# pierrepaleo/sift_pyocl

Hardware: AMD Instinct MI355X
Metric: SiftPlan.keypoints throughput, 4096x4096 fp32 (Mpix/s; keypoints/s in keypoints_per_s) (higher is better)
Workload: dtype f32

## Files before the change

sift_pyocl_amd/csrc/k_keypoint.hpp:

```cpp
#pragma once
#include <hip/hip_runtime.h>
#include <stdint.h>
#include "k_extrema.hpp"
#include "siftmath.hpp"

namespace siftk {

struct KpRecord { float x, y, scale, angle; uint8_t desc[128]; };
static_assert(sizeof(KpRecord) == 144, "record layout");

struct GradTaps { float xa, xb, ya, yb; bool bx, by; };

__device__ __forceinline__ GradTaps gradient_fetch(const float *__restrict__ I, int x, int y, int W, int H) {
    const size_t pos = (size_t)y * W + x;
    GradTaps t;
    t.bx = (x == 0) || (x == W - 1);
    t.by = (y == 0) || (y == H - 1);
    t.xa = I[x == W - 1 ? pos : pos + 1];
    t.xb = I[x == 0 ? pos : pos - 1];
    t.ya = I[y == 0 ? pos : pos - W];
    t.yb = I[y == H - 1 ? pos : pos + W];
    return t;
}

__device__ __forceinline__ void gradient_eval(const GradTaps &t, float &mag, float &ori) {
    float gx = t.xa - t.xb, gy = t.ya - t.yb;
    if (t.bx) gx = 2.0f * gx;
    if (t.by) gy = 2.0f * gy;
    mag = sqrtf(gx * gx + gy * gy);
    ori = siftmath::atan2f_(-gy, gx);
}

__device__ __forceinline__ void gradient_at(const float *__restrict__ I, int x, int y, int W, int H,
                                            float &mag, float &ori) {
    gradient_eval(gradient_fetch(I, x, y, W, H), mag, ori);
}

__device__ __forceinline__ int div_exact(int idx, int d, float inv, int &rem) {
    int q = (int)((float)idx * inv);
    rem = idx - q * d;
    if (rem < 0) { q--; rem += d; }
    else if (rem >= d) { q++; rem -= d; }
    return q;
}

#define SIFT_MAX_OCTAVES 24
#define SIFT_GROUPS 3
struct Counters {
    int n_rec;
    int tail_timeout;
    unsigned rec_word[SIFT_GROUPS];
    int g_kp[SIFT_GROUPS];
    int g_out[SIFT_GROUPS];
    int desc_next[SIFT_GROUPS];
    int n_cand[SIFT_MAX_OCTAVES + 1];
    int c_scale[SIFT_MAX_OCTAVES][3];
    int o_scale[SIFT_MAX_OCTAVES][3];
    uint32_t mm[2];
    int tail_ready[8];
};

struct OctaveTable {
    const float *base;
    long long off[SIFT_MAX_OCTAVES];
    int W[SIFT_MAX_OCTAVES], H[SIFT_MAX_OCTAVES];
    const float *gmap, *omap;
};
__device__ __forceinline__ size_t map_offset(const OctaveTable &tab, int oct, int scale) {
    return (size_t)(tab.off[oct] / 2) + (size_t)(scale - 1) * tab.W[oct] * tab.H[oct];
}

struct alignas(16) RecordSink {
    KpRecord *dev, *host;
    int dev_limit, host_limit;
};

__device__ __forceinline__ void descriptor_open(Counters *cnt, int group, int n, KpRecord *records, int rec_capacity, KpRecord *host_records,
                                                int host_capacity, RecordSink *S) {
    if (threadIdx.x == 0) {
        int base = 0;
        if (cnt) {
            if (blockIdx.x == 0) {
                base = atomicAdd(&cnt->n_rec, n);
                __hip_atomic_store(&cnt->rec_word[group], 0x80000000u | (unsigned)base, __ATOMIC_RELAXED, __HIP_MEMORY_SCOPE_AGENT);
            } else {
                unsigned w;
                while (!((w = __hip_atomic_load(&cnt->rec_word[group], __ATOMIC_RELAXED, __HIP_MEMORY_SCOPE_AGENT)) & 0x80000000u)) __builtin_amdgcn_s_sleep(16);
                base = (int)(w & 0x7fffffffu);
            }
        }
        S->dev = records + base; S->dev_limit = rec_capacity - base;
        S->host = host_records ? host_records + base : nullptr; S->host_limit = host_records ? host_capacity - base : 0;
    }
    __syncthreads();
}

__device__ __forceinline__ void store_record(const RecordSink *S, int i, const float4 kq, int b0, int b1, int lane, unsigned char *bytes) {
    bytes[lane] = (unsigned char)b0; bytes[lane + 64] = (unsigned char)b1;
    __builtin_amdgcn_wave_barrier();
    unsigned w = 0u;
    if (lane < 4) w = __float_as_uint(lane == 0 ? kq.x : (lane == 1 ? kq.y : (lane == 2 ? kq.z : kq.w)));
    else if (lane < 36) w = reinterpret_cast<const unsigned *>(bytes)[lane - 4];
    if (lane < 36) {
        const volatile RecordSink *v = S;
        if (i < v->dev_limit) reinterpret_cast<unsigned *>(v->dev + i)[lane] = w;
        if (i < v->host_limit) reinterpret_cast<unsigned *>(v->host + i)[lane] = w;
    }
    __builtin_amdgcn_wave_barrier();
}

__global__ void gather_records_kernel(const KpRecord *__restrict__ records, const int *__restrict__ idx, KpRecord *__restrict__ out, int n) {
    const long long total = (long long)n * 36;
    for (long long t = (long long)blockIdx.x * blockDim.x + threadIdx.x; t < total; t += (long long)gridDim.x * blockDim.x) {
        const int j = (int)(t / 36), w = (int)(t - (long long)j * 36);
        reinterpret_cast<unsigned *>(out + j)[w] = reinterpret_cast<const unsigned *>(records + idx[j])[w];
    }
}

#ifdef SIFT_PHASE_CLOCK
__device__ unsigned long long g_phase[32];
struct PhaseClock {
    unsigned long long t, t0;
    unsigned long long *acc;
    __device__ __forceinline__ void start(unsigned long long *lds16, int lane) {
        acc = lds16;
        if (lane < 16) lds16[lane] = 0ull;
        __builtin_amdgcn_wave_barrier();
        t0 = t = __builtin_amdgcn_s_memtime();
    }
    __device__ __forceinline__ void mark(int k, int lane) {
        const unsigned long long now = __builtin_amdgcn_s_memtime();
        if (lane == 0) (void)__hip_atomic_fetch_add(acc + k, now - t, __ATOMIC_RELAXED, __HIP_MEMORY_SCOPE_WORKGROUP);
        t = now;
    }
    __device__ __forceinline__ void count(int k, int lane) { if (lane == 0) (void)__hip_atomic_fetch_add(acc + k, 1ull, __ATOMIC_RELAXED, __HIP_MEMORY_SCOPE_WORKGROUP); }
    __device__ __forceinline__ void flush(int base, int lane) {
        const unsigned long long now = __builtin_amdgcn_s_memtime();
        if (lane == 0) acc[12] = now - t0;
        __builtin_amdgcn_wave_barrier();
        if (lane < 15) atomicAdd(&g_phase[base + lane], acc[lane]);
        if (lane == 15) atomicMax(&g_phase[base + 15], acc[12]);
    }
};
#define PH_MARK(k) ph.mark((k), lane)
#define PH_COUNT(k) ph.count((k), lane)
#define PH_WAIT_VM(n) asm volatile("s_waitcnt vmcnt(" #n ")" ::: "memory")
#else
#define PH_MARK(k)
#define PH_COUNT(k)
#define PH_WAIT_VM(n)
#endif

#define ABL(x) false

#define SIFT_ORI_OBUF 96
struct alignas(16) OriWaveLds {
    float pool[64 + 36 * 3 + 4];
    uint2 mask[36];
    unsigned mbase[36];
    float4 obuf[SIFT_ORI_OBUF];
    int oaux[SIFT_ORI_OBUF];
#ifdef SIFT_PHASE_CLOCK
    unsigned long long ph[16];
#endif
};

__device__ __forceinline__ int wave_prefix_incl(int x) {
    int t = x;
    t += __builtin_amdgcn_update_dpp(0, t, 0x111, 0xf, 0xf, false);
    t += __builtin_amdgcn_update_dpp(0, t, 0x112, 0xf, 0xf, false);
    t += __builtin_amdgcn_update_dpp(0, t, 0x114, 0xf, 0xf, false);
    t += __builtin_amdgcn_update_dpp(0, t, 0x118, 0xf, 0xf, false);
    t += __builtin_amdgcn_update_dpp(0, t, 0x142, 0xa, 0xf, false);
    t += __builtin_amdgcn_update_dpp(0, t, 0x143, 0xc, 0xf, false);
    return t;
}

template <bool MAPS>
__global__ __launch_bounds__(256) void orientation_kernel(OctaveTable tab, float ori_sigma,
                                                          const float4 *__restrict__ kp,
                                                          const int *__restrict__ kp_aux, Counters *cnt, int group,
                                                          int kp_capacity, float4 *__restrict__ okp,
                                                          int *__restrict__ oaux, int out_capacity, int team_below, int small_blocks) {
    __shared__ OriWaveLds lds_all[4];
    __shared__ double fold[36];
    __shared__ int s_hist[3 * SIFT_MAX_OCTAVES];
    const int lane = threadIdx.x & 63;
    OriWaveLds &L = lds_all[threadIdx.x >> 6];
    const int n = min(cnt->g_kp[group], kp_capacity);
    const int first = 0;
    const int count = n - first;
    const int nblocks = min((int)gridDim.x, count < 16384 ? small_blocks : (count < 65536 ? max(1024, small_blocks) : 4096));
    if ((int)blockIdx.x >= nblocks) return;
#ifdef SIFT_PHASE_CLOCK
    PhaseClock ph;
    ph.start(L.ph, lane);
#endif
    siftmath::load_atan_fold(fold);
    if (lane < 36) L.mask[lane] = make_uint2(0u, 0u);
    if (threadIdx.x < 3 * SIFT_MAX_OCTAVES) s_hist[threadIdx.x] = 0;
    __syncthreads();
    PH_MARK(0);
    const int wave = (blockIdx.x * blockDim.x + threadIdx.x) >> 6;
    const int nwaves = (nblocks * blockDim.x) >> 6;
    const float4 *pool4 = reinterpret_cast<const float4 *>(L.pool);
    __shared__ int s_pending[4], s_base;
    int pending = 0;
    auto store_pending = [&](int slot, int count) {
        __builtin_amdgcn_wave_barrier();
        for (int e = lane; e < count; e += 64)
            if (slot + e < out_capacity) { okp[slot + e] = L.obuf[e]; oaux[slot + e] = L.oaux[e]; }
        __builtin_amdgcn_wave_barrier();
    };
    auto flush_wave = [&]() {
        int slot = 0;
        if (lane == 0) slot = atomicAdd(&cnt->g_out[group], pending);
        store_pending(__shfl(slot, 0), pending);
        pending = 0;
    };
    const bool team = count < team_below;
    const int w4 = threadIdx.x >> 6;
    const int boff = team ? 64 * w4 : 0, bstep = team ? 256 : 64;
    for (int i = first + (team ? (int)blockIdx.x : wave); i < n; i += (team ? nblocks : nwaves)) {
        const float4 k = kp[i];
        const int aux = __builtin_amdgcn_readfirstlane(kp_aux[i]);
        const int scale = aux & 0xff, oct = aux >> 8;
        const int W = tab.W[oct], H = tab.H[oct], octsize = 1 << oct;
        if (!(k.y >= 0.0f)) continue;
        const float *I = tab.base + tab.off[oct] + (size_t)scale * W * H;
        const float *Gm = MAPS ? tab.gmap + map_offset(tab, oct, scale) : nullptr;
        const float *Om = MAPS ? tab.omap + map_offset(tab, oct, scale) : nullptr;
        auto taps_at = [&](int x, int y) {
            if (!MAPS) return gradient_fetch(I, x, y, W, H);
            GradTaps t = {};
            const size_t pos = (size_t)y * W + x;
            t.xa = Gm[pos]; t.xb = Om[pos];
            return t;
        };
        const int row = (int)((double)k.y + 0.5), col = (int)((double)k.z + 0.5);
        const float sigma = ori_sigma * k.w;
        const int radius = (int)((double)sigma * 3.0);
        const int rmin = max(0, row - radius), cmin = max(0, col - radius);
        const int rmax = min(row + radius, H - 2), cmax = min(col + radius, W - 2);
        const float lim = (float)(radius * radius) + 0.5f;
        const float two_s2 = 2.0f * sigma * sigma;
        const float r_two_s2 = 1.0f / two_s2;
        const bool fast_div = two_s2 >= 1e-3f && two_s2 <= 1e6f;
        const int wc = cmax - cmin + 1, hr = rmax - rmin + 1;
        const int total = (wc > 0 && hr > 0) ? wc * hr : 0;
        const float inv_wc = 1.0f / (float)max(wc, 1);
        float h = 0.0f;
        auto locate = [&](int base, int &r, int &c) {
            const int idx = base + lane;
            if (idx >= total) return false;
            int rem;
            const int q = div_exact(idx, wc, inv_wc, rem);
            r = rmin + q; c = cmin + rem;
            return true;
        };
        int nr = 0, nc = 0;
        bool nvalid = locate(boff, nr, nc);
        GradTaps ntaps = {};
        if (nvalid) ntaps = taps_at(nc, nr);
        PH_COUNT(13);
        PH_MARK(1);
        for (int base = 0; base < total; base += bstep) {
            bool valid = nvalid;
            const int r = nr, c = nc;
            const GradTaps taps = ntaps;
            nvalid = locate(base + bstep + boff, nr, nc);
            if (nvalid) ntaps = taps_at(nc, nr);
#ifdef SIFT_PHASE_CLOCK
            PH_COUNT(14);
            if (base + bstep + boff < total) PH_WAIT_VM(4); else PH_WAIT_VM(0);
            PH_MARK(2);
#endif
            int bin = 0;
            float val = 0.0f;
            if (valid) {
                float gx = taps.xa - taps.xb, gy = taps.ya - taps.yb;
                if (taps.bx) gx = 2.0f * gx;
                if (taps.by) gy = 2.0f * gy;
                const float gval = MAPS ? taps.xa : sqrtf(gx * gx + gy * gy);
                float dif = (float)r - k.y;
                float distsq = dif * dif;
                dif = (float)c - k.z;
                distsq = distsq + dif * dif;
                valid = (gval > 0.0f) && (distsq < lim);
                if (valid) {
                    const float earg = fast_div ? siftmath::div_by_reciprocal(-distsq, two_s2, r_two_s2) : -distsq / two_s2;
                    bool ok_a = true, ok_e;
                    float a = MAPS ? taps.xb : siftmath::atan2f_fast_try(-gy, gx, fold, ok_a);
                    float ew = siftmath::expf_fast_try(earg, ok_e);
                    if (!(ok_a && ok_e)) {
                        if (!MAPS && !ok_a) a = siftmath::atan2f_(-gy, gx);
                        if (!ok_e) ew = siftmath::expf_(earg);
                    }
                    bin = (int)siftmath::div_by_reciprocal(36.0f * (a + SM_PI_F + 0.001f), 2.0f * SM_PI_F, 1.0f / (2.0f * SM_PI_F));
                    valid = (bin >= 0) && (bin <= 36);
                    bin = min(max(bin, 0), 35);
                    val = ew * gval;
                }
                if (valid) atomicOr(reinterpret_cast<unsigned *>(L.mask) + 2 * bin + (lane >> 5), 1u << (lane & 31));
            }
            __builtin_amdgcn_wave_barrier();
            PH_MARK(3);
            const uint2 mine = (lane < 36) ? L.mask[lane] : make_uint2(0u, 0u);
            const int votes = __popc(mine.x) + __popc(mine.y);
            const int padded = (votes + 3) & ~3;
            const int seg = wave_prefix_incl(padded) - padded;
            if (lane < 36) L.mbase[lane] = (unsigned)seg;
            if (votes) reinterpret_cast<float4 *>(L.pool)[(seg + padded - 4) >> 2] = make_float4(0.f, 0.f, 0.f, 0.f);
            __builtin_amdgcn_wave_barrier();
            PH_MARK(4);
            {
                const uint2 mk = L.mask[bin];
                const unsigned mb = L.mbase[bin];
                const int pos = mb + __builtin_amdgcn_mbcnt_hi(mk.y, __builtin_amdgcn_mbcnt_lo(mk.x, 0u));
                if (valid) L.pool[pos] = val;
            }
            __builtin_amdgcn_wave_barrier();
            PH_MARK(5);
            if (!team) {
                for (int k0 = 0; k0 < padded; k0 += 4) {
                    const float4 v = pool4[(seg + k0) >> 2];
                    h = h + v.x; h = h + v.y; h = h + v.z; h = h + v.w;
                }
                if (votes) L.mask[lane] = make_uint2(0u, 0u);
                __builtin_amdgcn_wave_barrier();
                PH_MARK(6);
            } else {
                __syncthreads();
                if (w4 == 0 && lane < 36) {
#pragma unroll
                    for (int q = 0; q < 4; q++) {
                        const uint2 mq = lds_all[q].mask[lane];
                        const int vq = __popc(mq.x) + __popc(mq.y);
                        const int sq = (int)lds_all[q].mbase[lane];
                        const float4 *pq = reinterpret_cast<const float4 *>(lds_all[q].pool);
                        for (int k0 = 0; k0 < vq; k0 += 4) {
                            const float4 v = pq[(sq + k0) >> 2];
                            h = h + v.x; h = h + v.y; h = h + v.z; h = h + v.w;
                        }
                        if (vq) lds_all[q].mask[lane] = make_uint2(0u, 0u);
                    }
                }
                __syncthreads();
            }
        }
        if (team && w4 != 0) continue;
        const int lp = (lane == 0) ? 35 : lane - 1, ln = (lane >= 35) ? 0 : lane + 1;
        auto third = [&](float s) {
            return (__builtin_fabsf(s) >= 1e-25f && __builtin_fabsf(s) <= 1e30f) ? siftmath::div_by_reciprocal(s, 3.0f, 1.0f / 3.0f)
                                                                            : (float)((double)s / 3.0);
        };
#pragma unroll 1
        for (int pass = 0; pass < 6; pass++) {
            const float prev = __shfl(h, lp), nxt = __shfl(h, ln);
            float nh = third((prev + h) + nxt);
            const float nh0 = __shfl(nh, 0);
            if (lane == 35) nh = third((prev + h) + nh0);
            h = (lane < 36) ? nh : 0.0f;
        }
        float mx = (lane < 36) ? h : 0.0f;
#pragma unroll
        for (int off = 32; off > 0; off >>= 1) mx = fmaxf(mx, __shfl_xor(mx, off));
        const float maxval = fmaxf(mx, 0.0f);
        const uint64_t eq = __ballot(lane < 36 && h == maxval);
        const int argmax = (maxval > 0.0f && eq) ? (__ffsll((unsigned long long)eq) - 1) : 0;
        const float hp = __shfl(h, argmax == 0 ? 35 : argmax - 1);
        const float hn = __shfl(h, argmax == 35 ? 0 : argmax + 1);
        const float interp = 0.5f * (hp - hn) / (hp - 2.0f * maxval + hn);
        const float angle = 2.0f * SM_PI_F * ((float)argmax + 0.5f + interp) / 36.0f - SM_PI_F;
        const float hpp = __shfl(h, lp), hnn = __shfl(h, ln);
        bool extra = (lane < 36) && h > hpp && h > hnn && h >= 0.8f * maxval && lane != argmax;
        float a2 = 0.0f;
        if (extra) {
            const float it = 0.5f * (hpp - hnn) / (hpp - 2.0f * h + hnn);
            a2 = (float)((double)(2.0f * SM_PI_F * ((float)lane + 0.5f + it)) / 36.0 - (double)SM_PI_F);
            extra = (a2 >= -SM_PI_F) && (a2 <= SM_PI_F);
        }
        const uint64_t emask = __ballot(extra);
        const float ox = k.z * (float)octsize, oy = k.y * (float)octsize, os = k.w * (float)octsize;
        const float sum4 = ((ox + oy) + os) + angle;
        const int nmain = (sum4 == sum4) ? 1 : 0;
        const int nextra = __popcll((unsigned long long)emask);
        if (lane == 0) atomicAdd(&s_hist[3 * oct + min(max(scale - 1, 0), 2)], 1 + nextra);
        if (pending + nmain + nextra > SIFT_ORI_OBUF) flush_wave();
        if (lane == 0 && nmain) { L.obuf[pending] = make_float4(ox, oy, os, angle); L.oaux[pending] = aux; }
        if (extra) {
            const int at = pending + nmain + __popcll((unsigned long long)(emask & ((1ull << lane) - 1ull)));
            L.obuf[at] = make_float4(ox, oy, os, a2);
            L.oaux[at] = aux;
        }
        pending += nmain + nextra;
        PH_MARK(7);
    }
    if (lane == 0) s_pending[threadIdx.x >> 6] = pending;
    __syncthreads();
    if (threadIdx.x == 0) {
        const int tot = s_pending[0] + s_pending[1] + s_pending[2] + s_pending[3];
        s_base = tot ? atomicAdd(&cnt->g_out[group], tot) : 0;
    }
    __syncthreads();
    {
        const int w = threadIdx.x >> 6;
        int slot = s_base;
        for (int q = 0; q < w; q++) slot += s_pending[q];
        store_pending(slot, pending);
    }
    for (int t = threadIdx.x; t < 3 * SIFT_MAX_OCTAVES; t += blockDim.x)
        if (s_hist[t]) atomicAdd(&cnt->o_scale[0][0] + t, s_hist[t]);
#ifdef SIFT_PHASE_CLOCK
    PH_MARK(8);
    ph.flush(0, lane);
#endif
}


struct DescWaveLds {
    unsigned int mlo[128], mhi[128], mbase[128];
    float pool[8 * 64];
    int pool_cnt;
    int sij[128];
    float srx[128], scx[128];
    float V[128];
};

__global__ __launch_bounds__(256) __attribute__((amdgpu_waves_per_eu(4, 8))) void descriptor_stream_kernel(OctaveTable tab, const float4 *__restrict__ okp,
                                                         const int *__restrict__ oaux, Counters *cnt, int group,
                                                         int range_start, int range_end,
                                                         int out_capacity, KpRecord *__restrict__ records, int rec_capacity,
                                                         KpRecord *host_records, int host_capacity) {
    __shared__ DescWaveLds lds_all[4];
    __shared__ RecordSink sink;
    const int lane = threadIdx.x & 63, wave = threadIdx.x >> 6;
    DescWaveLds &L = lds_all[wave];
    int start = range_start, end = range_end;
    if (cnt) { start = 0; end = min(cnt->g_out[group], out_capacity); }
    descriptor_open(cnt, group, end, records, rec_capacity, host_records, host_capacity, &sink);
    L.mlo[lane] = 0u; L.mhi[lane] = 0u; L.mlo[lane + 64] = 0u; L.mhi[lane + 64] = 0u;
    if (lane == 0) L.pool_cnt = 0;
    const int gwave = blockIdx.x * 4 + wave, nwaves = gridDim.x * 4;
    const unsigned long long lt_mask = (1ull << lane) - 1ull;
    for (int i = start + gwave; i < end; i += nwaves) {
        const float4 kq = okp[i];
        const int aux = oaux[i];
        const int scale = aux & 0xff, oct = aux >> 8;
        const int W = tab.W[oct], H = tab.H[oct], octsize = 1 << oct;
        if (!(kq.y >= 0.0f)) {
            store_record(&sink, i, kq, 0, 0, lane, reinterpret_cast<unsigned char *>(L.V));
            continue;
        }
        const float *I = tab.base + tab.off[oct] + (size_t)scale * W * H;
        const float foct = (float)octsize;
        const float row = kq.y / foct, col = kq.x / foct, angle = kq.w;
        const int irow = (int)(row + 0.5f), icol = (int)(col + 0.5f);
        float sine, cosine;
        siftmath::sincosf_(angle, &sine, &cosine);
        const float spacing = kq.z / foct * 3.0f;
        const int iradius = (int)((1.414f * spacing * 2.5f) + 0.5f);
        const float drow = row - (float)irow, dcol = col - (float)icol;
        const int S = 2 * iradius + 1;
        const int total = S * S;
        const float inv_S = 1.0f / (float)S;
        float acc0 = 0.0f, acc1 = 0.0f;
        int list_n = 0, pos = 0;
        while (pos < total || list_n > 0) {
            while (list_n < 64 && pos < total) {
                const int idx = pos + lane;
                bool inside = false;
                float rx = 0.f, cx = 0.f;
                int ii = 0, jj = 0;
                if (idx < total) {
                    int rem;
                    const int q = div_exact(idx, S, inv_S, rem);
                    ii = q - iradius; jj = rem - iradius;
                    rx = ((cosine * (float)ii - sine * (float)jj) - drow) / spacing + 1.5f;
                    cx = ((sine * (float)ii + cosine * (float)jj) - dcol) / spacing + 1.5f;
                    const int yy = irow + ii, xx = icol + jj;
                    inside = rx > -1.0f && rx < 4.0f && cx > -1.0f && cx < 4.0f && yy >= 0 && yy < H && xx >= 0 && xx < W;
                }
                const unsigned long long bal = __ballot(inside);
                if (inside) {
                    const int at = list_n + __popcll(bal & lt_mask);
                    L.sij[at] = (ii + 32768) | ((jj + 32768) << 16);
                    L.srx[at] = rx;
                    L.scx[at] = cx;
                }
                list_n += __popcll(bal);
                pos += 64;
            }
            __builtin_amdgcn_wave_barrier();
            const int m = min(list_n, 64);
            int cbin[8];
            float cval[8];
#pragma unroll
            for (int n8 = 0; n8 < 8; n8++) { cbin[n8] = -1; cval[n8] = 0.0f; }
            if (lane < m && !ABL(3)) {
                const int pk = L.sij[lane];
                const int ii = (pk & 0xffff) - 32768, jj = ((pk >> 16) & 0xffff) - 32768;
                const float rx = L.srx[lane], cx = L.scx[lane];
                float g, o;
                if (ABL(2)) { g = I[(size_t)(irow + ii) * W + icol + jj]; o = g * 0.01f; }
                else gradient_at(I, icol + jj, irow + ii, W, H, g, o);
                const float er = rx - 1.5f, ec = cx - 1.5f;
                const float mag = g * (ABL(2) ? (er * ec) : siftmath::expf_(-0.125f * (er * er + ec * ec)));
                o = o - angle;
                while (o > 2.0f * SM_PI_F) o -= 2.0f * SM_PI_F;
                while (o < 0.0f) o += 2.0f * SM_PI_F;
                const float oval = 4.0f * o * SM_1_PI_F;
                const int ri = (int)((rx >= 0.0f) ? rx : rx - 1.0f);
                const int ci = (int)((cx >= 0.0f) ? cx : cx - 1.0f);
                const int oi = (int)((oval >= 0.0f) ? oval : oval - 1.0f);
                const float rf = rx - (float)ri, cf = cx - (float)ci, of = oval - (float)oi;
                const bool contributes = ri >= -1 && ri < 4 && oi >= 0 && oi <= 8 && rf >= 0.0f && rf <= 1.0f;
                if (contributes) {
                    const unsigned int bit = 1u << (lane & 31);
                    const int word = lane >> 5;
#pragma unroll
                    for (int a = 0; a < 2; a++) {
                        const int rb = ri + a;
                        const float rw = mag * (a == 0 ? 1.0f - rf : rf);
#pragma unroll
                        for (int bb = 0; bb < 2; bb++) {
                            const int cb = ci + bb;
                            const float cw = rw * (bb == 0 ? 1.0f - cf : cf);
                            const bool ok = rb >= 0 && rb < 4 && cb >= 0 && cb < 4;
#pragma unroll
                            for (int e = 0; e < 2; e++) {
                                int ob = oi + e;
                                const bool dup = (e == 1 && oi == 8);
                                if (ob >= 8) ob = 0;
                                const int n8 = a * 4 + bb * 2 + e;
                                if (ok && !dup) {
                                    cbin[n8] = (rb * 4 + cb) * 8 + ob;
                                    cval[n8] = cw * (e == 0 ? 1.0f - of : of);
                                    atomicOr((word ? L.mhi : L.mlo) + cbin[n8], bit);
                                }
                            }
                        }
                    }
                }
            }
            __builtin_amdgcn_wave_barrier();
            if (!(ABL(1) || ABL(3))) {
                const uint2 ia = make_uint2(L.mlo[lane], L.mhi[lane]), ib = make_uint2(L.mlo[lane + 64], L.mhi[lane + 64]);
                const int cnta = __popc(ia.x) + __popc(ia.y), cntb = __popc(ib.x) + __popc(ib.y);
                int base_a = 0;
                if (cnta + cntb) base_a = atomicAdd(&L.pool_cnt, cnta + cntb);
                const int base_b = base_a + cnta;
                if (cnta) L.mbase[lane] = (unsigned)base_a;
                if (cntb) L.mbase[lane + 64] = (unsigned)base_b;
                __builtin_amdgcn_wave_barrier();
                const unsigned lo_mask = (lane < 32) ? ((1u << lane) - 1u) : 0xffffffffu;
                const unsigned hi_mask = (lane < 32) ? 0u : ((1u << (lane - 32)) - 1u);
#pragma unroll
                for (int n8 = 0; n8 < 8; n8++)
                    if (cbin[n8] >= 0) {
                        const int b = cbin[n8];
                        L.pool[L.mbase[b] + __popc(L.mlo[b] & lo_mask) + __popc(L.mhi[b] & hi_mask)] = cval[n8];
                    }
                __builtin_amdgcn_wave_barrier();
                const int nmax = max(cnta, cntb);
                for (int r0 = 0; r0 < nmax; r0 += 4) {
                    float va[4], vb[4];
#pragma unroll
                    for (int u = 0; u < 4; u++) {
                        const float ra = L.pool[(base_a + r0 + u) & 511], rb_ = L.pool[(base_b + r0 + u) & 511];
                        va[u] = (r0 + u < cnta) ? ra : 0.0f;
                        vb[u] = (r0 + u < cntb) ? rb_ : 0.0f;
                    }
#pragma unroll
                    for (int u = 0; u < 4; u++) { acc0 = acc0 + va[u]; acc1 = acc1 + vb[u]; }
                }
                __builtin_amdgcn_wave_barrier();
                if (cnta) { L.mlo[lane] = 0u; L.mhi[lane] = 0u; }
                if (cntb) { L.mlo[lane + 64] = 0u; L.mhi[lane + 64] = 0u; }
                if (lane == 0) L.pool_cnt = 0;
            } else {
                L.mlo[lane] = 0u; L.mhi[lane] = 0u; L.mlo[lane + 64] = 0u; L.mhi[lane + 64] = 0u;
            }
            __builtin_amdgcn_wave_barrier();
            const int rest = list_n - m;
            int mij = 0; float mrx = 0.f, mcx = 0.f;
            if (lane < rest) { mij = L.sij[m + lane]; mrx = L.srx[m + lane]; mcx = L.scx[m + lane]; }
            __builtin_amdgcn_wave_barrier();
            if (lane < rest) { L.sij[lane] = mij; L.srx[lane] = mrx; L.scx[lane] = mcx; }
            list_n = rest;
            __builtin_amdgcn_wave_barrier();
        }
        L.V[lane] = acc0; L.V[lane + 64] = acc1;
        __builtin_amdgcn_wave_barrier();
        float norm = 0.0f;
#pragma unroll 8
        for (int k2 = 0; k2 < 128; k2++) { const float t = L.V[k2]; norm = norm + t * t; }
        norm = 1.0f / sqrtf(norm);
        acc0 = acc0 * norm; acc1 = acc1 * norm;
        const bool ch = (acc0 > 0.2f) || (acc1 > 0.2f);
        if (acc0 > 0.2f) acc0 = 0.2f;
        if (acc1 > 0.2f) acc1 = 0.2f;
        __builtin_amdgcn_wave_barrier();
        L.V[lane] = acc0; L.V[lane + 64] = acc1;
        __builtin_amdgcn_wave_barrier();
        if (__ballot(ch)) {
            float n2 = 0.0f;
#pragma unroll 8
            for (int k2 = 0; k2 < 128; k2++) { const float t = L.V[k2]; n2 = n2 + t * t; }
            n2 = 1.0f / sqrtf(n2);
            acc0 = acc0 * n2; acc1 = acc1 * n2;
        }
        __builtin_amdgcn_wave_barrier();
        const int i0 = (acc0 == acc0) ? (int)(512.0 * (double)acc0) : 0;
        const int i1 = (acc1 == acc1) ? (int)(512.0 * (double)acc1) : 0;
        store_record(&sink, i, kq, min(255, i0), min(255, i1), lane, reinterpret_cast<unsigned char *>(L.V));
    }
}

__global__ void gradient_kernel(const float *__restrict__ img, float *__restrict__ grad, float *__restrict__ ori, int W, int H) {
    const int x = blockIdx.x * blockDim.x + threadIdx.x, y = blockIdx.y;
    if (x >= W || y >= H) return;
    float g, o;
    gradient_at(img, x, y, W, H, g, o);
    grad[(size_t)y * W + x] = g;
    ori[(size_t)y * W + x] = o;
}

#define SIFT_MAP_ROWS 32
__host__ __device__ inline long long gradient_map_items_of(int W, int H) {
    return 3LL * ((H + SIFT_MAP_ROWS - 1) / SIFT_MAP_ROWS) * ((W + 255) / 256);
}
__global__ __launch_bounds__(256) void gradient_maps_kernel(OctaveTable tab, int oct_lo, int oct_hi, long long total,
                                                            float *__restrict__ gmap, float *__restrict__ omap) {
    __shared__ double fold[36];
    siftmath::load_atan_fold(fold);
    __syncthreads();
    for (long long item = blockIdx.x; item < total; item += gridDim.x) {
        long long rem = item;
        int oct = oct_lo;
        while (oct < oct_hi - 1 && rem >= gradient_map_items_of(tab.W[oct], tab.H[oct])) { rem -= gradient_map_items_of(tab.W[oct], tab.H[oct]); oct++; }
        const int W = tab.W[oct], H = tab.H[oct];
        const int nx = (W + 255) / 256, nyp = (H + SIFT_MAP_ROWS - 1) / SIFT_MAP_ROWS;
        const int plane = (int)(rem / ((long long)nyp * nx));
        const int r2 = (int)(rem - (long long)plane * nyp * nx);
        const int cy = r2 / nx, xb = r2 - cy * nx;
        if (plane > 2) continue;
        const int x = xb * 256 + (int)threadIdx.x;
        if (x >= W) continue;
        const float *I = tab.base + tab.off[oct] + (size_t)(plane + 1) * W * H;
        const size_t mo = map_offset(tab, oct, plane + 1);
        const int y1 = min((cy + 1) * SIFT_MAP_ROWS, H);
        for (int y = cy * SIFT_MAP_ROWS; y < y1; y++) {
            const GradTaps t = gradient_fetch(I, x, y, W, H);
            float gx = t.xa - t.xb, gy = t.ya - t.yb;
            if (t.bx) gx = 2.0f * gx;
            if (t.by) gy = 2.0f * gy;
            bool ok;
            float a = siftmath::atan2f_fast_try(-gy, gx, fold, ok);
            if (!ok) a = siftmath::atan2f_(-gy, gx);
            gmap[mo + (size_t)y * W + x] = sqrtf(gx * gx + gy * gy);
            omap[mo + (size_t)y * W + x] = a;
        }
    }
}

__global__ void math_kernel(int fn, const float *__restrict__ a, const float *__restrict__ bb, float *__restrict__ out, int64_t n) {
    __shared__ double fold[36];
    siftmath::load_atan_fold(fold);
    __syncthreads();
    const int64_t stride = (int64_t)gridDim.x * blockDim.x;
    for (int64_t i = (int64_t)blockIdx.x * blockDim.x + threadIdx.x; i < n; i += stride) {
        float s, c;
        switch (fn) {
            case 0: out[i] = siftmath::expf_(a[i]); break;
            case 1: out[i] = siftmath::exp2f_(a[i]); break;
            case 2: siftmath::sincosf_(a[i], &s, &c); out[i] = s; break;
            case 3: siftmath::sincosf_(a[i], &s, &c); out[i] = c; break;
            case 5: out[i] = siftmath::expf_fast(a[i]); break;
            case 6: out[i] = siftmath::atan2f_fast(a[i], bb[i], fold); break;
            case 7: out[i] = siftmath::div_by_reciprocal(a[i], bb[i], 1.0f / bb[i]); break;
            default: out[i] = siftmath::atan2f_(a[i], bb[i]); break;
        }
    }
}

}
```

Measured before the change: 21650.

## Iterate only in-circle pixels via per-row interval table in orientation kernel

Builds a per-row table of column intervals inside the circular window (rows up to 128), so each wave only visits pixels that pass the distance test instead of the whole bounding square. Positions are decoded with readlane scans over packed row words. It also adds an optional two-pixels-per-lane mode, off by default, which widens the LDS mask to uint4. This cuts wasted lanes and gradient fetches for pixels outside the circle, at the cost of table-building and scalar scan overhead, plus larger LDS masks.

```diff
diff --git a/sift_pyocl_amd/csrc/k_keypoint.hpp b/sift_pyocl_amd/csrc/k_keypoint.hpp
--- a/sift_pyocl_amd/csrc/k_keypoint.hpp
+++ b/sift_pyocl_amd/csrc/k_keypoint.hpp
@@ -154,9 +154,13 @@
 #define ABL(x) false
 
 #define SIFT_ORI_OBUF 96
+#define SIFT_ORI_ROWS 128
+#ifndef SIFT_ORI_TWO
+#define SIFT_ORI_TWO 0
+#endif
 struct alignas(16) OriWaveLds {
-    float pool[64 + 36 * 3 + 4];
-    uint2 mask[36];
+    float pool[64 * (1 + SIFT_ORI_TWO) + 36 * 3 + 4];
+    uint4 mask[36];
     unsigned mbase[36];
     float4 obuf[SIFT_ORI_OBUF];
     int oaux[SIFT_ORI_OBUF];
@@ -174,6 +178,25 @@
     t += __builtin_amdgcn_update_dpp(0, t, 0x142, 0xa, 0xf, false);
     t += __builtin_amdgcn_update_dpp(0, t, 0x143, 0xc, 0xf, false);
     return t;
+}
+
+__device__ __forceinline__ bool ori_row_interval(int r, float ky, float kz, float lim, int &first, int &end) {
+    const float dy = (float)r - ky;
+    const float a = dy * dy;
+    first = end = 0;
+    if (!(a < lim) || !(kz == kz)) return true;
+    auto P = [&](int c) {
+        const float d = (float)c - kz;
+        const float q = a + d * d;
+        return q < lim;
+    };
+    const float x = sqrtf(lim - a);
+    const int el = (int)__builtin_floorf(kz - x), er = (int)__builtin_floorf(kz + x) + 1;
+    const bool out_l = !P(el), out_r = !P(er), in_l = P(el + 1), in_r = P(er - 1);
+    const bool full = out_l && out_r && in_l && in_r;
+    first = el + 1;
+    end = full ? er : el + 1;
+    return full || (el + 1 == er && out_l && out_r);
 }
 
 template <bool MAPS>
@@ -197,7 +220,7 @@
     ph.start(L.ph, lane);
 #endif
     siftmath::load_atan_fold(fold);
-    if (lane < 36) L.mask[lane] = make_uint2(0u, 0u);
+    if (lane < 36) L.mask[lane] = make_uint4(0u, 0u, 0u, 0u);
     if (threadIdx.x < 3 * SIFT_MAX_OCTAVES) s_hist[threadIdx.x] = 0;
     __syncthreads();
     PH_MARK(0);
@@ -219,8 +242,9 @@
         pending = 0;
     };
     const bool team = count < team_below;
-    const int w4 = threadIdx.x >> 6;
-    const int boff = team ? 64 * w4 : 0, bstep = team ? 256 : 64;
+    const int w4 = __builtin_amdgcn_readfirstlane(threadIdx.x >> 6);
+    const bool two = SIFT_ORI_TWO && !team;
+    const int boff = team ? 64 * w4 : 0, bstep = team ? 256 : (two ? 128 : 64);
     for (int i = first + (team ? (int)blockIdx.x : wave); i < n; i += (team ? nblocks : nwaves)) {
         const float4 k = kp[i];
         const int aux = __builtin_amdgcn_readfirstlane(kp_aux[i]);
@@ -240,43 +264,81 @@
         const int row = (int)((double)k.y + 0.5), col = (int)((double)k.z + 0.5);
         const float sigma = ori_sigma * k.w;
         const int radius = (int)((double)sigma * 3.0);
-        const int rmin = max(0, row - radius), cmin = max(0, col - radius);
-        const int rmax = min(row + radius, H - 2), cmax = min(col + radius, W - 2);
+        const int rmin = __builtin_amdgcn_readfirstlane(max(0, row - radius)), cmin = __builtin_amdgcn_readfirstlane(max(0, col - radius));
+        const int rmax = __builtin_amdgcn_readfirstlane(min(row + radius, H - 2)), cmax = __builtin_amdgcn_readfirstlane(min(col + radius, W - 2));
         const float lim = (float)(radius * radius) + 0.5f;
         const float two_s2 = 2.0f * sigma * sigma;
         const float r_two_s2 = 1.0f / two_s2;
         const bool fast_div = two_s2 >= 1e-3f && two_s2 <= 1e6f;
         const int wc = cmax - cmin + 1, hr = rmax - rmin + 1;
-        const int total = (wc > 0 && hr > 0) ? wc * hr : 0;
+        int total = (wc > 0 && hr > 0) ? wc * hr : 0;
         const float inv_wc = 1.0f / (float)max(wc, 1);
         float h = 0.0f;
-        auto locate = [&](int base, int &r, int &c) {
-            const int idx = base + lane;
-            if (idx >= total) return false;
-            int rem;
-            const int q = div_exact(idx, wc, inv_wc, rem);
-            r = rmin + q; c = cmin + rem;
-            return true;
+        bool tabled = !MAPS && !team && hr <= SIFT_ORI_ROWS && wc <= SIFT_ORI_ROWS && radius < (1 << 20) && total > 0;
+        unsigned tb0 = ~0u, tb1 = ~0u;
+        if (tabled) {
+            int carry = 0;
+            bool ok = true;
+            for (int r0 = 0; r0 < hr; r0 += 64) {
+                const int rr = r0 + lane;
+                int c_first, c_end;
+                ok = ori_row_interval(rmin + rr, k.y, k.z, lim, c_first, c_end) && ok;
+                c_first = max(c_first, cmin);
+                int c = min(c_end - 1, cmax) - c_first + 1;
+                if (rr >= hr || c < 0) c = 0;
+                const int incl = wave_prefix_incl(c);
+                const unsigned word = rr < hr ? ((unsigned)(carry + incl - c) << 14) | ((unsigned)rr << 7) | (unsigned)(c ? c_first - cmin : 0) : ~0u;
+                if (r0 == 0) tb0 = word; else tb1 = word;
+                carry += __builtin_amdgcn_readlane(incl, 63);
+            }
+            tabled = !__ballot(!ok);
+            if (tabled) total = carry;
+        }
+        auto row_word = [&](int j) {
+            return j < 64 ? __builtin_amdgcn_readlane(tb0, j) : __builtin_amdgcn_readlane(tb1, j - 64);
         };
-        int nr = 0, nc = 0;
-        bool nvalid = locate(boff, nr, nc);
-        GradTaps ntaps = {};
-        if (nvalid) ntaps = taps_at(nc, nr);
-        PH_COUNT(13);
-        PH_MARK(1);
-        for (int base = 0; base < total; base += bstep) {
-            bool valid = nvalid;
-            const int r = nr, c = nc;
-            const GradTaps taps = ntaps;
-            nvalid = locate(base + bstep + boff, nr, nc);
-            if (nvalid) ntaps = taps_at(nc, nr);
-#ifdef SIFT_PHASE_CLOCK
-            PH_COUNT(14);
-            if (base + bstep + boff < total) PH_WAIT_VM(4); else PH_WAIT_VM(0);
-            PH_MARK(2);
-#endif
-            int bin = 0;
-            float val = 0.0f;
+        const int hr64 = min(hr, 64);
+        auto scan = [&](unsigned stop, unsigned key, unsigned &w, unsigned &last, int &j) {
+            for (; j < hr64; j++) {
+                const unsigned wj = __builtin_amdgcn_readlane(tb0, j);
+                if (wj >= stop) return;
+                w = wj <= key ? wj : w;
+                last = wj;
+            }
+            for (; j < hr; j++) {
+                const unsigned wj = __builtin_amdgcn_readlane(tb1, j - 64);
+                if (wj >= stop) return;
+                w = wj <= key ? wj : w;
+                last = wj;
+            }
+        };
+        int jrow = 0;
+        auto locate = [&](int b, int &ra, int &ca, bool &va, int &rb, int &cb, bool &vb) {
+            const int sa = b + lane, sb = sa + 64;
+            va = sa < total; vb = two && sb < total;
+            if (b >= total) return;
+            if (tabled) {
+                int j = jrow + 1;
+                while (j < hr && (row_word(j) >> 14) <= (unsigned)b) j++;
+                unsigned last = row_word(j - 1), wa = last;
+                scan((unsigned)(b + 64) << 14, ((unsigned)sa << 14) | 0x3fffu, wa, last, j);
+                unsigned wb = last;
+                if (two) scan((unsigned)(b + 128) << 14, ((unsigned)sb << 14) | 0x3fffu, wb, last, j);
+                jrow = j - 1;
+                ra = rmin + (int)((wa >> 7) & 127u); ca = min(cmin + (int)(wa & 127u) + (sa - (int)(wa >> 14)), cmax);
+                rb = rmin + (int)((wb >> 7) & 127u); cb = min(cmin + (int)(wb & 127u) + (sb - (int)(wb >> 14)), cmax);
+            } else {
+                int rem;
+                int q = div_exact(min(sa, total - 1), wc, inv_wc, rem);
+                ra = rmin + q; ca = cmin + rem;
+                if (two) {
+                    q = div_exact(min(sb, total - 1), wc, inv_wc, rem);
+                    rb = rmin + q; cb = cmin + rem;
+                }
+            }
+        };
+        auto evaluate = [&](bool valid, int r, int c, const GradTaps &taps, int half, int &bin, float &val) {
+            bin = 0; val = 0.0f;
             if (valid) {
                 float gx = taps.xa - taps.xb, gy = taps.ya - taps.yb;
                 if (taps.bx) gx = 2.0f * gx;
@@ -301,12 +363,40 @@
                     bin = min(max(bin, 0), 35);
                     val = ew * gval;
                 }
-                if (valid) atomicOr(reinterpret_cast<unsigned *>(L.mask) + 2 * bin + (lane >> 5), 1u << (lane & 31));
-            }
+                if (valid) atomicOr(reinterpret_cast<unsigned *>(L.mask) + 4 * bin + 2 * half + (lane >> 5), 1u << (lane & 31));
+            }
+            return valid;
+        };
+        int nra = 0, nca = 0, nrb = 0, ncb = 0;
+        bool nva = false, nvb = false;
+        locate(boff, nra, nca, nva, nrb, ncb, nvb);
+        GradTaps ntaps_a = {}, ntaps_b = {};
+        if (nva) ntaps_a = taps_at(nca, nra);
+        if (SIFT_ORI_TWO && nvb) ntaps_b = taps_at(ncb, nrb);
+        PH_COUNT(13);
+        PH_MARK(1);
+        for (int base = 0; base < total; base += bstep) {
+            const bool va = nva, vb = nvb;
+            const int ra = nra, ca = nca, rb = nrb, cb = ncb;
+            const GradTaps taps_a = ntaps_a, taps_b = ntaps_b;
+            nva = false; nvb = false;
+            locate(base + bstep + boff, nra, nca, nva, nrb, ncb, nvb);
+            if (nva) ntaps_a = taps_at(nca, nra);
+            if (SIFT_ORI_TWO && nvb) ntaps_b = taps_at(ncb, nrb);
+#ifdef SIFT_PHASE_CLOCK
+            PH_COUNT(14);
+            if (base + bstep + boff < total) PH_WAIT_VM(8); else PH_WAIT_VM(0);
+            PH_MARK(2);
+#endif
+            int bin_a, bin_b;
+            float val_a, val_b;
+            const bool valid_a = evaluate(va, ra, ca, taps_a, 0, bin_a, val_a);
+            const bool valid_b = SIFT_ORI_TWO ? evaluate(vb, rb, cb, taps_b, 1, bin_b, val_b) : false;
+            if (!SIFT_ORI_TWO) { bin_b = 0; val_b = 0.0f; }
             __builtin_amdgcn_wave_barrier();
             PH_MARK(3);
-            const uint2 mine = (lane < 36) ? L.mask[lane] : make_uint2(0u, 0u);
-            const int votes = __popc(mine.x) + __popc(mine.y);
+            const uint4 mine = (lane < 36) ? L.mask[lane] : make_uint4(0u, 0u, 0u, 0u);
+            const int votes = (__popc(mine.x) + __popc(mine.y)) + (__popc(mine.z) + __popc(mine.w));
             const int padded = (votes + 3) & ~3;
             const int seg = wave_prefix_incl(padded) - padded;
             if (lane < 36) L.mbase[lane] = (unsigned)seg;
@@ -314,10 +404,12 @@
             __builtin_amdgcn_wave_barrier();
             PH_MARK(4);
             {
-                const uint2 mk = L.mask[bin];
-                const unsigned mb = L.mbase[bin];
-                const int pos = mb + __builtin_amdgcn_mbcnt_hi(mk.y, __builtin_amdgcn_mbcnt_lo(mk.x, 0u));
-                if (valid) L.pool[pos] = val;
+                const uint4 ma = L.mask[bin_a], mb = L.mask[bin_b];
+                const unsigned sa = L.mbase[bin_a], sb = L.mbase[bin_b];
+                const int pos_a = sa + __builtin_amdgcn_mbcnt_hi(ma.y, __builtin_amdgcn_mbcnt_lo(ma.x, 0u));
+                const int pos_b = sb + (__popc(mb.x) + __popc(mb.y)) + __builtin_amdgcn_mbcnt_hi(mb.w, __builtin_amdgcn_mbcnt_lo(mb.z, 0u));
+                if (valid_a) L.pool[pos_a] = val_a;
+                if (SIFT_ORI_TWO && valid_b) L.pool[pos_b] = val_b;
             }
             __builtin_amdgcn_wave_barrier();
             PH_MARK(5);
@@ -326,7 +418,7 @@
                     const float4 v = pool4[(seg + k0) >> 2];
                     h = h + v.x; h = h + v.y; h = h + v.z; h = h + v.w;
                 }
-                if (votes) L.mask[lane] = make_uint2(0u, 0u);
+                if (votes) L.mask[lane] = make_uint4(0u, 0u, 0u, 0u);
                 __builtin_amdgcn_wave_barrier();
                 PH_MARK(6);
             } else {
@@ -334,15 +426,15 @@
                 if (w4 == 0 && lane < 36) {
 #pragma unroll
                     for (int q = 0; q < 4; q++) {
-                        const uint2 mq = lds_all[q].mask[lane];
-                        const int vq = __popc(mq.x) + __popc(mq.y);
+                        const uint4 mq = lds_all[q].mask[lane];
+                        const int vq = (__popc(mq.x) + __popc(mq.y)) + (__popc(mq.z) + __popc(mq.w));
                         const int sq = (int)lds_all[q].mbase[lane];
                         const float4 *pq = reinterpret_cast<const float4 *>(lds_all[q].pool);
                         for (int k0 = 0; k0 < vq; k0 += 4) {
                             const float4 v = pq[(sq + k0) >> 2];
                             h = h + v.x; h = h + v.y; h = h + v.z; h = h + v.w;
                         }
-                        if (vq) lds_all[q].mask[lane] = make_uint2(0u, 0u);
+                        if (vq) lds_all[q].mask[lane] = make_uint4(0u, 0u, 0u, 0u);
                     }
                 }
                 __syncthreads();
```

Result: no change. 21500 (-0.7%).
